# sxontheway/milliEye

Hardware: AMD Instinct MI355X
Metric: frames/sec YOLOv3-416+fusion @batch32, 1/2/4/8 MI355X; mAP@0.5 vs ref (higher is better)
Workload: dtype f32; 1 GPU; yolov3.cfg 416x416 fp32 inference, batch=32 per GPU, full milliEye: Darknet.forward -> NMS -> Network.forward mode 0 (R-CNN head + radar fusion, 2 radar boxes/frame) -> output rows, synthetic frames U[0,1), deterministic trained-like weights; stage=full, batch_per_gpu=32, global_batch=32, img_size=416, parallelism=frames sharded over 1 GPU(s), one process per GPU, no data-path collective, rccl_ranks=0, full=False, output_rows_last_step=6449, rois_last_step=6449

## Files before the change

### millieye_amd/csrc/common.h

```cpp
#pragma once
#include <hip/hip_runtime.h>
#include <stdint.h>
#include <stdio.h>
#include <stdlib.h>
#include "millieye_hip.h"

namespace me {

void set_error(const char* fmt, ...);

inline int check_launch(const char* what) {
  hipError_t e = hipGetLastError();
  if (e != hipSuccess) {
    set_error("%s: %s", what, hipGetErrorString(e));
    return (int)e;
  }
  return 0;
}

inline bool aligned16(const void* p) { return (reinterpret_cast<uintptr_t>(p) & 15u) == 0; }

inline int64_t ceil_div(int64_t a, int64_t b) { return (a + b - 1) / b; }

inline int store_mode() {
  static const int mode = [] {
    const char* e = getenv("MILLIEYE_STORE_MODE");
    return e ? atoi(e) : 0;
  }();
  return mode;
}

inline int epilogue16() {
  static const int on = [] {
    const char* e = getenv("MILLIEYE_EPILOGUE16");
    return e ? atoi(e) != 0 : 1;
  }();
  return on;
}

typedef unsigned st_u32x4 __attribute__((ext_vector_type(4)));
__device__ __forceinline__ void store16(void* ptr, uint4 v, int mode) {
  if (mode == 0) {
    *reinterpret_cast<uint4*>(ptr) = v;
  } else {
    st_u32x4 d = {v.x, v.y, v.z, v.w};
    if (mode == 1)
      asm volatile("global_store_dwordx4 %0, %1, off nt\n\ts_nop 1" ::"v"(ptr), "v"(d) : "memory");
    else
      asm volatile("global_store_dwordx4 %0, %1, off sc1\n\ts_nop 1" ::"v"(ptr), "v"(d) : "memory");
  }
}
__device__ __forceinline__ void store4(float* ptr, float v, int mode) {
  if (mode == 0)
    *ptr = v;
  else
    __builtin_nontemporal_store(v, ptr);
}

inline me_yolo_rect_desc yolo_rect_of(const me_yolo_desc& s) {
  me_yolo_rect_desc r;
  r.x = s.x;
  r.out = s.out;
  r.x_pitch = s.x_pitch;
  r.n = s.n;
  r.gh = r.gw = s.g;
  r.num_anchors = s.num_anchors;
  r.num_classes = s.num_classes;
  r.rows_total = s.rows_total;
  r.row_offset = s.row_offset;
  r.stride = s.stride;
  for (int i = 0; i < 16; ++i) r.anchors[i] = s.anchors[i];
  return r;
}

}

#define ME_REQUIRE(cond, code, ...)   \
  do {                                \
    if (!(cond)) {                    \
      me::set_error(__VA_ARGS__);     \
      return (code);                  \
    }                                 \
  } while (0)

#define ME_HIP(call)                                                 \
  do {                                                               \
    hipError_t e__ = (call);                                         \
// ... 6 lines not shown
```

### millieye_amd/csrc/conv.hip

```cpp
#include <stdlib.h>

#include "common.h"
#include "dma.h"

#include "conv32_common.h"

namespace me32 {
int launch_p8_tile(const ConvP& p, int tile, hipStream_t stream);
bool ws1x1_f32_eligible(const ConvP& p);
int launch_ws1x1_f32(const ConvP& p, hipStream_t stream);
bool ws3x3_f32_eligible(const ConvP& p);
int launch_ws3x3_f32(const ConvP& p, hipStream_t stream);
bool stem_mfma_eligible(const ConvP& p);
int launch_stem_mfma(const ConvP& p, hipStream_t stream);
}

namespace {

template <int BM, int BN, int BK, int WR, int WC, int ABL = 0, int PRIO = 0>
__global__ __launch_bounds__(256) void conv_igemm_f32(ConvP p) {
  static_assert(WR * WC == 4, "4 waves per workgroup");
  constexpr int TM = BM / WR, TN = BN / WC;
  constexpr int MT = TM / 32, NT = TN / 32;
  static_assert(MT >= 1 && NT >= 1, "wave tile must hold at least one 32x32 MFMA tile");
// ... 426 lines not shown
    for (int kx = 0; kx < 3; ++kx) {
      const int iy = oy * p.stride - p.pad + ky, ix = ox * p.stride - p.pad + kx;
      const bool ok = ((unsigned)iy < (unsigned)p.h) && ((unsigned)ix < (unsigned)p.w);
#pragma unroll
      for (int c = 0; c < 3; ++c) {
        float v = 0.f;
        if (ok)
          v = p.x_nchw ? p.x[(((long long)nimg * 3 + c) * p.h + iy) * p.w + ix]
                       : p.x[((long long)(nimg * p.h + iy) * p.w + ix) * p.x_pitch + c];
        xin[(ky * 3 + kx) * 3 + c] = v;
      }
    }
  const float* __restrict__ wg = p.wgt + (long long)co0 * K;
  float acc[CT];
#pragma unroll
  for (int j = 0; j < CT; ++j) {
    float a = 0.f;
#pragma unroll
    for (int k = 0; k < K; ++k) a = fmaf(xin[k], wg[j * K + k], a);
    acc[j] = apply_act(a * p.scale[co0 + j] + p.shift[co0 + j], p.act);
  }
  float* yrow = p.y + (long long)m * p.y_pitch + co0;
#pragma unroll
  for (int j = 0; j < CT; j += 4) *reinterpret_cast<float4*>(yrow + j) = make_float4(acc[j], acc[j + 1], acc[j + 2], acc[j + 3]);
}

using namespace me_dma;

__device__ __forceinline__ unsigned udiv_magic32(unsigned n, unsigned m, unsigned s) { return (__umulhi(n, m) + n) >> s; }

template <int N, class F, int I = 0>
__device__ __forceinline__ void static_for(F&& f) {
  if constexpr (I < N) {
    f(std::integral_constant<int, I>{});
    static_for<N, F, I + 1>(static_cast<F&&>(f));
  }
}

__device__ __forceinline__ void tile_coords(const ConvP& p, int t, int& tile_m, int& tile_n) {
  const int per_panel = p.tiles_m * p.gn;
  const int panel = t / per_panel;
  const int r = t - panel * per_panel;
  const int left = p.tiles_n - panel * p.gn;
  const int width = left < p.gn ? left : p.gn;
  tile_m = r / width;
  tile_n = panel * p.gn + (r - tile_m * width);
}

constexpr int buf_min_waves(int bm, int bn, int wr, int wc, int minw, bool hyb_or_masked) {
  const int per_wave = (bm / wr) * (bn / wc);
  return minw != 1 ? minw : per_wave == 1024 ? 6 : per_wave == 2048 && hyb_or_masked ? 4 : 1;
}

template <int BM, int BN, int WR, int WC, int MINW = 1, int BABL = 0, int HYB = 0, int KORD = 0, int DEEP = 0, int MASKED = 0>
__global__ __launch_bounds__(64 * WR * WC, buf_min_waves(BM, BN, WR, WC, MINW, HYB || MASKED)) void conv_igemm_buf_f32(ConvP p) {
  constexpr int NW = WR * WC;
  static_assert(NW == 4 || NW == 8, "4 or 8 waves per workgroup");
  constexpr int BK = 16, NST = DEEP ? (KORD ? 9 : 6) : 3;
  constexpr int DEPTH = NST - 1;
  constexpr int TM = BM / WR, TN = BN / WC;
  constexpr int MT = TM / 32, NT = TN / 32;
  constexpr int GA = BM / 16, G = (BM + BN) / 16;
  constexpr int LPW = (G + NW - 1) / NW;
  constexpr int LA = GA / NW;
  constexpr int STAGE_F = LPW * NW * 256;
  static_assert(GA % NW == 0, "A groups must split evenly over the waves");

  extern __shared__ __attribute__((aligned(16))) float smem[];
  const unsigned lds_base = (unsigned)(unsigned long long)(__attribute__((address_space(3))) float*)smem;

  const int tid = threadIdx.x;
  const int lane = tid & 63;
  const int wave = __builtin_amdgcn_readfirstlane(tid >> 6);
  const int wr = wave / WC, wc = wave % WC;
  const int r32 = lane & 31, hh = lane >> 5;

  int tile_m, tile_n;
  int sid = blockIdx.y;
  int piece = -1;
  {
    int nwg = p.tiles_m * p.tiles_n;
    int bid = blockIdx.x;
    int first = 0, per = 1;
    if constexpr (HYB) {
      if (bid < p.bulk) {
        nwg = p.bulk;
      } else {
        bid -= p.bulk;
        first = p.bulk;
        per = p.splitk;
        nwg = (nwg - p.bulk) * p.splitk;
      }
    }
    const int q = nwg >> 3, r = nwg & 7;
    const int xcd = bid & 7, idx = bid >> 3;
    int wg = (xcd < r ? xcd * (q + 1) : r * (q + 1) + (xcd - r) * q) + idx;
    if constexpr (HYB) {
      if (first || p.bulk == 0) {
        piece = wg;
        sid = wg % per;
        wg = first + wg / per;
      } else {
        sid = 0;
      }
    }
    tile_coords(p, wg, tile_m, tile_n);
    tile_m = __builtin_amdgcn_readfirstlane(tile_m);
    tile_n = __builtin_amdgcn_readfirstlane(tile_n);
  }
  const int m0 = tile_m * BM, n0 = tile_n * BN;
  const int hw = p.ho * p.wo;

  const int img0 = (int)udiv_magic32((unsigned)m0, p.hw_m, p.hw_s);
  const long long img_elems = (long long)p.h * p.w * p.x_pitch;
  const long long bias_elems = ((long long)p.pad * p.w + p.pad) * p.x_pitch;
  const u32x4 rsrc_a = make_rsrc(p.x + (long long)img0 * img_elems - bias_elems);
  const bool b_tiled = p.wgt_tiled != nullptr;
  const u32x4 rsrc_b = make_rsrc(b_tiled ? p.wgt_tiled + (long long)n0 * 16 : p.wgt + (long long)n0 * p.ktot);
  const unsigned b_row = b_tiled ? 64u : (unsigned)p.ktot * 4u;
  const unsigned b_step = b_tiled ? (unsigned)p.cout * 64u : BK * 4u;

  const int lrow = lane >> 2;
  unsigned v_base[LPW];
  constexpr bool KS3 = KORD == 1;
  unsigned v_pad[LA];
  unsigned v_cur[LPW];
#pragma unroll
  for (int j = 0; j < LPW; ++j) {
    const int g = wave + NW * j;
    const int row = g * 16 + lrow;
    const int q = (lane & 3) ^ ((row >> 2) & 3);
    v_base[j] = kOobOffset;
    if (j < LA) {
      unsigned padmask = 0xFFFFFFFFu;
      const int m = m0 + row;
      if (m < p.M) {
        const int nimg = (int)udiv_magic32((unsigned)m, p.hw_m, p.hw_s);
        const int rem = m - nimg * hw;
        const int oy = (int)udiv_magic32((unsigned)rem, p.wo_m, p.wo_s), ox = rem - oy * p.wo;
        const int iy0 = oy * p.stride - p.pad, ix0 = ox * p.stride - p.pad;
        unsigned ok = 0;
        auto in_w = [&](int kx) { return (unsigned)(ix0 + kx) < (unsigned)p.w ? 1u : 0u; };
        auto in_h = [&](int ky) { return (unsigned)(iy0 + ky) < (unsigned)p.h; };
        if (KS3 || p.ks == 3) {
          const unsigned cols = in_w(0) | in_w(1) << 1 | in_w(2) << 2;
          ok = (in_h(0) ? cols : 0u) | (in_h(1) ? cols << 3 : 0u) | (in_h(2) ? cols << 6 : 0u);
        } else if (p.ks == 1) {
          ok = in_h(0) ? in_w(0) : 0u;
        } else {
          unsigned cols = 0;
          for (int kx = 0; kx < p.ks; ++kx) cols |= in_w(kx) << kx;
          for (int ky = 0; ky < p.ks; ++ky) ok |= (in_h(ky) ? cols : 0u) << (ky * p.ks);
        }
        padmask = ~ok;
        const long long e = (long long)(nimg - img0) * img_elems + ((long long)iy0 * p.w + ix0) * p.x_pitch + bias_elems;
        v_base[j] = (unsigned)(e * 4) + 16u * q;
      }
      v_pad[j] = padmask;
    } else if (g < G) {
      const int co_local = row - BM;
      if (n0 + co_local < p.cout) v_base[j] = (unsigned)co_local * b_row + 16u * q;
    }
    v_cur[j] = BABL == 1 ? kOobOffset : v_base[j];
  }

  int s_begin = sid * p.sps;
  int s_end = (s_begin + p.sps < p.stages) ? s_begin + p.sps : p.stages;
  if constexpr (HYB) {
    if (piece < 0) {
      s_begin = 0;
      s_end = p.stages;
    }
  }
  f32x16 acc[MT][NT];
#pragma unroll
  for (int i = 0; i < MT; ++i)
#pragma unroll
    for (int j = 0; j < NT; ++j)
#pragma unroll
      for (int e = 0; e < 16; ++e) acc[i][j][e] = 0.f;

  constexpr unsigned STAGE_B = STAGE_F * 4u;
  const unsigned wave_lds = __builtin_amdgcn_readfirstlane(lds_base + (unsigned)wave * 1024u);
  const unsigned pitch4 = (unsigned)p.x_pitch * 4u;
  const int sw = (r32 >> 2) & 3;
  const int off0 = ((0 + hh) ^ sw) * 4, off1 = ((2 + hh) ^ sw) * 4;
  const float* a_frag = smem + (wr * TM + r32) * BK;
  const float* b_frag = smem + (BM + wc * TN + r32) * BK;

  auto compute_stage = [&](const float* Ab, const float* Bb) {
    if (MT * NT >= 4) __builtin_amdgcn_s_setprio(1);
    float4 af[2][MT], bf[2][NT];
#pragma unroll
    for (int half = 0; half < 2; ++half) {
      const int off = half ? off1 : off0;
#pragma unroll
      for (int i = 0; i < MT; ++i) af[half][i] = *reinterpret_cast<const float4*>(Ab + i * 32 * BK + off);
#pragma unroll
      for (int j = 0; j < NT; ++j) bf[half][j] = *reinterpret_cast<const float4*>(Bb + j * 32 * BK + off);
    }
    __builtin_amdgcn_sched_barrier(0);
#pragma unroll
    for (int half = 0; half < 2; ++half) {
#pragma unroll
      for (int kk = 0; kk < 4; ++kk)
#pragma unroll
        for (int i = 0; i < MT; ++i)
#pragma unroll
          for (int j = 0; j < NT; ++j) {
            const float4 av = af[half][i], bv = bf[half][j];
            const float a = kk == 0 ? av.x : kk == 1 ? av.y : kk == 2 ? av.z : av.w;
            const float b = kk == 0 ? bv.x : kk == 1 ? bv.y : kk == 2 ? bv.z : bv.w;
            acc[i][j] = __builtin_amdgcn_mfma_f32_32x32x2f32(a, b, acc[i][j], 0, 0, 0);
          }
    }
    if (MT * NT >= 4) __builtin_amdgcn_s_setprio(0);
  };

  if constexpr (KORD == 0) {
    int tap = 0, cc = 0, ky = 0, kx = 0;
    unsigned tmask = 0xFFFFFFFFu;
    if constexpr (MASKED) {
      tmask = p.tapmask[n0 / p.mask_cols] & ((1u << (p.ks * p.ks)) - 1u);
      tap = __builtin_ctz(tmask);
      ky = tap / p.ks;
      kx = tap - ky * p.ks;
      s_begin = 0;
      s_end = __builtin_popcount(tmask) * p.cs;
    } else if (s_begin != 0) {
      tap = s_begin / p.cs;
      cc = s_begin - tap * p.cs;
      ky = tap / p.ks;
      kx = tap - ky * p.ks;
    }
    unsigned a_off = 0, b_off = 0;
    auto enter_tap = [&]() {
#pragma unroll
      for (int j = 0; j < LA; ++j) v_cur[j] = (BABL == 1 || ((v_pad[j] >> (MASKED ? (tap & 31) : tap)) & 1u)) ? kOobOffset : v_base[j];
      a_off = (unsigned)(ky * p.w + kx) * pitch4;
      b_off = (unsigned)tap * (unsigned)p.cs * b_step;
    };
    enter_tap();
    a_off += (unsigned)cc * (BK * 4u);
    b_off += (unsigned)cc * b_step;
    auto issue_stage = [&](unsigned lds_dst) {
      dma_stage<LPW, LA, NW * 1024>(v_cur, rsrc_a, rsrc_b, __builtin_amdgcn_readfirstlane(a_off),
                                    __builtin_amdgcn_readfirstlane(b_off), lds_dst);
      a_off += BK * 4u;
      b_off += b_step;
      if (++cc == p.cs) {
        cc = 0;
        do {
          ++tap;
          if (++kx == p.ks) {
            kx = 0;
            ++ky;
          }
        } while (MASKED && tap < p.ks * p.ks && !((tmask >> tap) & 1u));
        enter_tap();
      }
    };
    const int nstages = s_end - s_begin;
    for (int i = 0; i < DEPTH && i < nstages; ++i) issue_stage(wave_lds + (unsigned)i * STAGE_B);
    auto wait_landed = [&](int younger) {
      bool done = false;
      static_for<DEPTH>([&](auto r_c) {
        constexpr int R = decltype(r_c)::value;
        if (!done && younger <= R) {
          asm volatile("s_waitcnt vmcnt(%0) lgkmcnt(0)" ::"n"(LPW * R) : "memory");
          done = true;
        }
      });
      if (!done) asm volatile("s_waitcnt vmcnt(%0) lgkmcnt(0)" ::"n"(LPW * (DEPTH - 1)) : "memory");
    };
    auto step = [&](auto slot_c) {
      constexpr int SLOT = decltype(slot_c)::value;
      asm volatile("s_waitcnt vmcnt(%0) lgkmcnt(0)" ::"n"(LPW * (DEPTH - 1)) : "memory");
      __builtin_amdgcn_s_barrier();
      asm volatile("" ::: "memory");
      issue_stage(wave_lds + ((SLOT + DEPTH) % NST) * STAGE_B);
      compute_stage(a_frag + SLOT * STAGE_F, b_frag + SLOT * STAGE_F);
    };
    int s = 0;
    for (; s + NST <= nstages - DEPTH; s += NST) static_for<NST>(step);
    int slot = 0;
    for (; s < nstages; ++s) {
      wait_landed(nstages - 1 - s);
      __builtin_amdgcn_s_barrier();
      asm volatile("" ::: "memory");
      if (s + DEPTH < nstages) issue_stage(wave_lds + (slot == 0 ? NST - 1 : slot - 1) * STAGE_B);
      compute_stage(a_frag + slot * STAGE_F, b_frag + slot * STAGE_F);
      slot = slot == NST - 1 ? 0 : slot + 1;
    }
  } else {
    unsigned v_tap[9][LPW];
    unsigned a_tap[9], b_tap[9];
#pragma unroll
    for (int t = 0; t < 9; ++t) {
#pragma unroll
      for (int j = 0; j < LPW; ++j)
        v_tap[t][j] = j < LA ? ((BABL == 1 || ((v_pad[j < LA ? j : 0] >> t) & 1u)) ? kOobOffset : v_base[j]) : v_cur[j];
      a_tap[t] = (unsigned)((t / 3) * p.w + (t % 3)) * pitch4;
      b_tap[t] = (unsigned)t * (unsigned)p.cs * b_step;
    }
    const int c_begin = s_begin / 9, c_end = s_end / 9;
    unsigned ca = (unsigned)c_begin * (BK * 4u), cb = (unsigned)c_begin * b_step;
    auto issue = [&](auto tap_c, unsigned ca_, unsigned cb_, unsigned lds_dst) {
      constexpr int T = decltype(tap_c)::value;
      dma_stage<LPW, LA, NW * 1024>(v_tap[T], rsrc_a, rsrc_b, __builtin_amdgcn_readfirstlane(a_tap[T] + ca_),
                                    __builtin_amdgcn_readfirstlane(b_tap[T] + cb_), lds_dst);
    };
    auto step = [&](auto tap_c, auto last_c) {
      constexpr int T = decltype(tap_c)::value;
      constexpr bool LAST = decltype(last_c)::value;
      constexpr int SLOT = T % NST;
      constexpr int YOUNGER = (LAST && 8 - T < DEPTH - 1) ? 8 - T : DEPTH - 1;
      asm volatile("s_waitcnt vmcnt(%0) lgkmcnt(0)" ::"n"(LPW * YOUNGER) : "memory");
      __builtin_amdgcn_s_barrier();
      asm volatile("" ::: "memory");
      constexpr unsigned DST = ((SLOT + DEPTH) % NST) * STAGE_B;
      if constexpr (T + DEPTH < 9)
        issue(std::integral_constant<int, (T + DEPTH) % 9>{}, ca, cb, wave_lds + DST);
      else if constexpr (!LAST)
        issue(std::integral_constant<int, (T + DEPTH) % 9>{}, ca + BK * 4u, cb + b_step, wave_lds + DST);
      compute_stage(a_frag + SLOT * STAGE_F, b_frag + SLOT * STAGE_F);
    };
    auto chunk = [&](auto last_c) { static_for<9>([&](auto tap_c) { step(tap_c, last_c); }); };
    static_for<DEPTH>([&](auto tap_c) { issue(tap_c, ca, cb, wave_lds + decltype(tap_c)::value * STAGE_B); });
    for (int c = c_begin; c + 1 < c_end; ++c) {
      chunk(std::false_type{});
      ca += BK * 4u;
      cb += b_step;
    }
    chunk(std::true_type{});
  }

  const bool split = HYB ? piece >= 0 : p.splitk > 1;
  if (split) {
    const long long slab_stride = HYB ? (long long)(BM * BN) : (long long)p.M * p.cout;
    float* slab0 = HYB ? p.partial + (long long)(piece - sid) * (BM * BN) : p.partial;
    auto slab_index = [&](int i, int j, int e, long long& idx) {
      const int lm = wr * TM + i * 32 + (e & 3) + 8 * (e >> 2) + 4 * hh, lc = wc * TN + j * 32 + r32;
      if (HYB) {
        idx = (long long)lm * BN + lc;
        return true;
      }
      idx = (long long)(m0 + lm) * p.cout + (n0 + lc);
      return m0 + lm < p.M && n0 + lc < p.cout;
    };
    float* mine = slab0 + (long long)sid * slab_stride;
#pragma unroll
    for (int j = 0; j < NT; ++j)
#pragma unroll
      for (int i = 0; i < MT; ++i)
#pragma unroll
        for (int e = 0; e < 16; ++e) {
          long long idx;
          if (!slab_index(i, j, e, idx)) continue;
          if (p.counters)
            __hip_atomic_store(mine + idx, acc[i][j][e], __ATOMIC_RELAXED, __HIP_MEMORY_SCOPE_AGENT);
          else
            mine[idx] = acc[i][j][e];
        }
    if (p.counters == nullptr) return;
    asm volatile("s_waitcnt vmcnt(0)" ::: "memory");
    __syncthreads();
    int* last_flag = reinterpret_cast<int*>(smem);
    if (tid == 0) {
      int* cnt = p.counters + (HYB ? piece / p.splitk : tile_m * p.tiles_n + tile_n);
      const int ticket = __hip_atomic_fetch_add(cnt, 1, __ATOMIC_RELAXED, __HIP_MEMORY_SCOPE_AGENT);
      const int last = ticket == p.splitk - 1;
      if (last) __hip_atomic_store(cnt, 0, __ATOMIC_RELAXED, __HIP_MEMORY_SCOPE_AGENT);
      *last_flag = last;
    }
    __syncthreads();
    if (*last_flag == 0) return;
#pragma unroll
    for (int j = 0; j < NT; ++j)
#pragma unroll
      for (int i = 0; i < MT; ++i)
#pragma unroll
        for (int e = 0; e < 16; ++e) {
          long long idx;
          if (!slab_index(i, j, e, idx)) continue;
          float a = __hip_atomic_load(slab0 + idx, __ATOMIC_RELAXED, __HIP_MEMORY_SCOPE_AGENT);
// ... 385 lines not shown
      attr_set = true;
    }
  }
  const long long blocks = (long long)p.tiles_m * p.tiles_n;
  ME_REQUIRE(blocks < (1ll << 31), ME_E_TOOBIG, "me_conv2d_f32: grid too large");
  hipLaunchKernelGGL(kern, dim3((unsigned)blocks, (unsigned)p.splitk), dim3(256), lds, stream, p);
  int rc = me::check_launch("conv_igemm_f32");
  if (rc || p.splitk == 1) return rc;
  long long rb = ((long long)p.M * p.cout + 255) / 256;
  if (rb > 256 * 16) rb = 256 * 16;
  hipLaunchKernelGGL(conv_splitk_reduce_f32, dim3((unsigned)rb), dim3(256), 0, stream, p);
  return me::check_launch("conv_splitk_reduce_f32");
}

template <int BM, int BN, int WR, int WC, int DPRIO = 0, int MINW = 1, int DABL = 0>
int launch_dma(ConvP& p, hipStream_t stream) {
  ME_REQUIRE(p.ks * p.ks <= 32, ME_E_BADARG, "conv_igemm_dma_f32: filters larger than 5x5 need the register-staged tiles (51-55)");
  constexpr int BK = 16;
  p.cs = (p.cin + BK - 1) / BK;
  p.stages = p.ks * p.ks * p.cs;
  p.tiles_m = (p.M + BM - 1) / BM;
  p.tiles_n = (p.cout + BN - 1) / BN;
  plan_split(p);
  constexpr int NW = WR * WC;
  constexpr int LPW = ((BM + BN) / 16 + NW - 1) / NW;
  const size_t lds = (size_t)3 * LPW * NW * 256 * sizeof(float);
  auto kern = conv_igemm_dma_f32<BM, BN, WR, WC, DPRIO, MINW, DABL>;
  if (lds > 64 * 1024) {
    static bool attr_set = false;
    if (!attr_set) {
      ME_HIP(hipFuncSetAttribute(reinterpret_cast<const void*>(kern), hipFuncAttributeMaxDynamicSharedMemorySize,
                                 (int)lds));
      attr_set = true;
    }
  }
  const long long blocks = (long long)p.tiles_m * p.tiles_n;
  ME_REQUIRE(blocks < (1ll << 31), ME_E_TOOBIG, "me_conv2d_f32: grid too large");
  hipLaunchKernelGGL(kern, dim3((unsigned)blocks, (unsigned)p.splitk), dim3(64 * NW), lds, stream, p);
  int rc = me::check_launch("conv_igemm_dma_f32");
  if (rc || p.splitk == 1) return rc;
  long long rb = ((long long)p.M * p.cout + 255) / 256;
  if (rb > 256 * 16) rb = 256 * 16;
  hipLaunchKernelGGL(conv_splitk_reduce_f32, dim3((unsigned)rb), dim3(256), 0, stream, p);
  return me::check_launch("conv_splitk_reduce_f32");
}

template <int BM>
bool buf_addressable(const ConvP& p) {
  if (p.cin % 16 != 0 || p.x_nchw) return false;
  const long long hw = (long long)p.ho * p.wo;
  const long long span_imgs = (BM - 1) / hw + 2;
  const long long img_bytes = (long long)p.h * p.w * p.x_pitch * 4;
  const long long tap_bytes = ((long long)p.ks * p.w + p.ks) * p.x_pitch * 4 + (long long)p.cin * 4;
  const long long a_max = span_imgs * img_bytes + 2 * tap_bytes;
  const long long b_max = 256ll * p.ktot * 4 + (long long)p.ktot * 4;
  const long long b_tiled_max = p.wgt_tiled ? (long long)p.ktot * p.cout * 4 + 256ll * 64 : 0;
  return a_max < (1ll << 31) && b_max < (1ll << 31) && b_tiled_max < (1ll << 31) && (long long)p.x_pitch * 4 < (1ll << 31);
}

void magic_u32(unsigned d, unsigned* m, unsigned* s) {
  unsigned sh = 0;
  while ((1ull << sh) < d) ++sh;
  *s = sh;
  *m = (unsigned)(((1ull << 32) * ((1ull << sh) - d)) / d + 1);
}

template <int BN>
void choose_order(ConvP& p) {
  static const long long kPanelBytes = [] {
    const char* e = getenv("MILLIEYE_PANEL_KB");
    return (e && atoi(e) > 0 ? (long long)atoi(e) : 1300ll) * 1024;
  }();
  static const int kChunkMajor = [] {
    const char* e = getenv("MILLIEYE_KORD");
    return e ? atoi(e) : 2;
  }();
  const long long col_bytes = (long long)BN * p.ktot * 4;
  p.gn = p.tiles_n;
  p.kord = (p.ks == 3 && p.cs >= 4 && kChunkMajor == 2) ? 1 : 0;
  if (col_bytes * p.tiles_n > kPanelBytes) {
    const long long fit = kPanelBytes / col_bytes;
    p.gn = fit < 1 ? 1 : fit > p.tiles_n ? p.tiles_n : (int)fit;
    if (p.ks == 3 && kChunkMajor >= 1) p.kord = 1;
  }
}

template <int BM, int BN, int WR, int WC, int MINW, int BABL, int HYB, int KORD, int DEEP = 0, int MASKED = 0>
int launch_buf_kernel(const ConvP& p, dim3 grid, hipStream_t stream) {
  constexpr int NW = WR * WC;
  constexpr int LPW = ((BM + BN) / 16 + NW - 1) / NW;
  constexpr int NST = DEEP ? (KORD ? 9 : 6) : 3;
  const size_t lds = (size_t)NST * LPW * NW * 256 * sizeof(float);
  auto kern = conv_igemm_buf_f32<BM, BN, WR, WC, MINW, BABL, HYB, KORD, DEEP, MASKED>;
  if (lds > 64 * 1024) {
    static bool attr_set = false;
    if (!attr_set) {
      ME_HIP(hipFuncSetAttribute(reinterpret_cast<const void*>(kern), hipFuncAttributeMaxDynamicSharedMemorySize,
                                 (int)lds));
      attr_set = true;
    }
  }
  hipLaunchKernelGGL(kern, grid, dim3(64 * NW), lds, stream, p);
  return me::check_launch(HYB ? "conv_igemm_buf_f32<tail split>" : "conv_igemm_buf_f32");
}

template <int BM, int BN, int WR, int WC, int MINW = 1, int BABL = 0, int DEEP = 0>
int launch_buf(ConvP& p, hipStream_t stream) {
  if (p.ks * p.ks > 32) {
    if constexpr (WR * WC == 4)
      return launch_igemm<BM, BN, 16, WR, WC>(p, stream);
    else
      return launch_igemm<128, 128, 16, 2, 2>(p, stream);
  }
  if (p.mask_cols)
    ME_REQUIRE(buf_addressable<BM>(p) && p.mask_cols % BN == 0 && BABL == 0 && DEEP == 0, ME_E_BADARG,
               "me_conv2d_f32: tap masks need cin %% 16 == 0, offsets below 2^31 and a tile width (%d) that divides tap_mask_cols", BN);
  if (!buf_addressable<BM>(p)) return launch_dma<BM, BN, WR, WC, 1, MINW>(p, stream);
  constexpr int BK = 16;
  p.cs = (p.cin + BK - 1) / BK;
  p.stages = p.ks * p.ks * p.cs;
  p.tiles_m = (p.M + BM - 1) / BM;
  p.tiles_n = (p.cout + BN - 1) / BN;
  choose_order<BN>(p);
  if (BABL || p.mask_cols) p.kord = 0;
  plan_split(p);
  const long long blocks = (long long)p.tiles_m * p.tiles_n;
  ME_REQUIRE(blocks < (1ll << 31), ME_E_TOOBIG, "me_conv2d_f32: grid too large");
  const dim3 grid((unsigned)blocks, (unsigned)p.splitk);
  if (blocks > p.counters_len || p.splitk == 1) p.counters = nullptr;
  int rc;
  if constexpr (BABL == 0) {
    if (p.mask_cols) {
      if constexpr (DEEP == 0) rc = launch_buf_kernel<BM, BN, WR, WC, MINW, 0, 0, 0, 0, 1>(p, grid, stream);
      else rc = ME_E_BADARG;
    } else
      rc = p.kord ? launch_buf_kernel<BM, BN, WR, WC, MINW, 0, 0, 1, DEEP>(p, grid, stream)
                  : launch_buf_kernel<BM, BN, WR, WC, MINW, 0, 0, 0, DEEP>(p, grid, stream);
  } else {
    rc = launch_buf_kernel<BM, BN, WR, WC, MINW, BABL, 0, 0>(p, grid, stream);
  }
  if (rc || p.splitk == 1 || p.counters) return rc;
  long long rb = ((long long)p.M * p.cout + 255) / 256;
  if (rb > 256 * 16) rb = 256 * 16;
  hipLaunchKernelGGL(conv_splitk_reduce_f32, dim3((unsigned)rb), dim3(256), 0, stream, p);
  return me::check_launch("conv_splitk_reduce_f32");
}

template <int BM, int BN, int WR, int WC, int MINW = 1, int DEEP = 0>
int launch_buf_tail(ConvP& p, hipStream_t stream, long long ws_bytes) {
  ME_REQUIRE(p.ks * p.ks <= 32 && buf_addressable<BM>(p), ME_E_BADARG,
             "me_conv2d_f32: the tail-split tiles need cin %% 16 == 0 and offsets below 2^31");
  constexpr int BK = 16;
  p.cs = (p.cin + BK - 1) / BK;
  p.stages = p.ks * p.ks * p.cs;
  p.tiles_m = (p.M + BM - 1) / BM;
  p.tiles_n = (p.cout + BN - 1) / BN;
  choose_order<BN>(p);
  const long long tiles = (long long)p.tiles_m * p.tiles_n;
  ME_REQUIRE(tiles < (1ll << 24), ME_E_TOOBIG, "me_conv2d_f32: grid too large");
  plan_split(p);
  p.bulk = (int)(tiles / 256 * 256);
  const long long tail = tiles - p.bulk;
  if (tail == 0 || p.splitk <= 1) {
    p.splitk = 1;
    p.bulk = 0;
    return launch_buf<BM, BN, WR, WC, MINW, 0, DEEP>(p, stream);
  }
  const long long need = tail * p.splitk * BM * BN * (long long)sizeof(float);
  ME_REQUIRE(p.partial && ws_bytes >= need, ME_E_BADARG, "me_conv2d_f32: tail split %d needs a workspace of %lld bytes",
             p.splitk, need);
  const dim3 grid((unsigned)(p.bulk + tail * p.splitk));
  if (tail > p.counters_len) p.counters = nullptr;
  int rc = p.kord ? launch_buf_kernel<BM, BN, WR, WC, MINW, 0, 1, 1, DEEP>(p, grid, stream)
                  : launch_buf_kernel<BM, BN, WR, WC, MINW, 0, 1, 0, DEEP>(p, grid, stream);
  if (rc || p.counters) return rc;
  long long rb = (tail * BM * BN + 255) / 256;
  if (rb > 256 * 16) rb = 256 * 16;
  hipLaunchKernelGGL(conv_tail_reduce_f32, dim3((unsigned)rb), dim3(256), 0, stream, p, BM, BN);
  return me::check_launch("conv_tail_reduce_f32");
}

int fill_params(const me_conv_desc* d, ConvP& p) {
  p.store_mode = me::store_mode();
  ME_REQUIRE(d != nullptr, ME_E_NULLPTR, "me_conv2d_f32: null descriptor");
  ME_REQUIRE(d->n > 0 && d->h > 0 && d->w > 0 && d->cin > 0 && d->cout > 0, ME_E_BADARG,
             "me_conv2d_f32: non-positive dimension");
  ME_REQUIRE(d->ksize >= 1 && d->stride >= 1 && d->pad >= 0, ME_E_BADARG, "me_conv2d_f32: bad ksize/stride/pad");
  const int ho = (d->h + 2 * d->pad - d->ksize) / d->stride + 1;
  const int wo = (d->w + 2 * d->pad - d->ksize) / d->stride + 1;
  ME_REQUIRE(ho == d->ho && wo == d->wo, ME_E_BADARG, "me_conv2d_f32: ho/wo (%d,%d) != derived (%d,%d)", d->ho,
             d->wo, ho, wo);
  ME_REQUIRE((long long)d->n * d->ho * d->wo < (1ll << 31), ME_E_TOOBIG, "me_conv2d_f32: too many output pixels");
  p.x = d->x; p.wgt = d->wgt; p.wgt_tiled = d->wgt_tiled; p.scale = d->scale; p.shift = d->shift; p.res = d->res; p.y = d->y;
  p.x_pitch = d->x_pitch; p.res_pitch = d->res_pitch; p.y_pitch = d->y_pitch;
  p.n = d->n; p.h = d->h; p.w = d->w; p.cin = d->cin; p.cout = d->cout; p.ks = d->ksize;
  p.stride = d->stride; p.pad = d->pad; p.ho = d->ho; p.wo = d->wo; p.act = d->act; p.ups = d->upsample;
  p.x_nchw = d->x_nchw;
  p.M = d->n * d->ho * d->wo;
  p.ktot = d->ksize * d->ksize * d->cin;
  magic_u32((unsigned)(d->ho * d->wo), &p.hw_m, &p.hw_s);
  magic_u32((unsigned)d->wo, &p.wo_m, &p.wo_s);
  p.cs = p.stages = p.tiles_m = p.tiles_n = p.bulk = p.gn = p.kord = 0;
  p.partial = nullptr;
  p.splitk = 1;
  p.sps = 0;
  p.counters = d->tile_counters_len > 0 ? d->tile_counters : nullptr;
  p.counters_len = p.counters ? d->tile_counters_len : 0;
  p.mask_cols = d->tap_mask_cols > 0 ? d->tap_mask_cols : 0;
  for (int i = 0; i < 4; ++i) p.tapmask[i] = d->tap_mask[i];
  auto rows16 = [](const float* ptr, long long pitch) { return me::aligned16(ptr) && pitch % 4 == 0 && pitch < (1ll << 22); };
  p.ep16 = me::epilogue16() && d->upsample == 1 && d->act != ME_ACT_SIGMOID && rows16(d->y, d->y_pitch) &&
           (!d->res || rows16(d->res, d->res_pitch)) && me::aligned16(d->scale) && me::aligned16(d->shift);
  return 0;
}

}

extern "C" {

int64_t me_conv2d_flops(const me_conv_desc* d) {
  if (!d) return 0;
  return 2ll * d->n * d->ho * d->wo * (int64_t)d->cout * d->ksize * d->ksize * d->cin;
}

int64_t me_conv2d_workspace_bytes(const me_conv_desc* d) {
  ConvP p;
  if (!d || fill_params(d, p) != 0 || d->cin <= 4) return 0;
// ... 145 lines not shown
```

### millieye_amd/csrc/dma.h

```cpp
#pragma once
#include <hip/hip_runtime.h>

namespace me_dma {

typedef unsigned u32x4 __attribute__((ext_vector_type(4)));
constexpr unsigned kOobOffset = 0x80000000u;

__device__ __forceinline__ u32x4 make_rsrc(const void* base) {
  const unsigned long long b = (unsigned long long)base;
  u32x4 r;
  r.x = __builtin_amdgcn_readfirstlane((unsigned)b);
  r.y = __builtin_amdgcn_readfirstlane((unsigned)(b >> 32) & 0xffffu);
  r.z = kOobOffset;
  r.w = 0x00020000u;
  return r;
}

template <int LPW, int LA, int STEP>
__device__ __forceinline__ void dma_stage(const unsigned (&v)[LPW], u32x4 ra, u32x4 rb, unsigned sa, unsigned sb,
                                          unsigned dst) {
  static_assert(LPW >= 2 && LPW <= 4 && LA >= 1 && LA <= 2, "unsupported DMA shape");
#define ME_DMA_HEAD "s_mov_b32 m0, %[d]\n\ts_nop 0\n\t"
#define ME_DMA_NEXT "s_add_u32 m0, m0, %[st]\n\ts_nop 0\n\t"
#define ME_DMA_A(i) "buffer_load_dwordx4 %[v" #i "], %[ra], %[sa] offen lds\n\t"
#define ME_DMA_B(i) "buffer_load_dwordx4 %[v" #i "], %[rb], %[sb] offen lds\n\t"
#define ME_DMA_TAIL ""
  if constexpr (LPW == 4 && LA == 2) {
    asm volatile(ME_DMA_HEAD ME_DMA_A(0) ME_DMA_NEXT ME_DMA_A(1) ME_DMA_NEXT ME_DMA_B(2) ME_DMA_NEXT ME_DMA_B(3) ME_DMA_TAIL
                 :
                 : [d] "s"(dst), [st] "n"(STEP), [ra] "s"(ra), [rb] "s"(rb), [sa] "s"(sa), [sb] "s"(sb), [v0] "v"(v[0]),
                   [v1] "v"(v[1]), [v2] "v"(v[2]), [v3] "v"(v[3])
                 : "memory", "scc");
  } else if constexpr (LPW == 3 && LA == 2) {
    asm volatile(ME_DMA_HEAD ME_DMA_A(0) ME_DMA_NEXT ME_DMA_A(1) ME_DMA_NEXT ME_DMA_B(2) ME_DMA_TAIL
                 :
                 : [d] "s"(dst), [st] "n"(STEP), [ra] "s"(ra), [rb] "s"(rb), [sa] "s"(sa), [sb] "s"(sb), [v0] "v"(v[0]),
                   [v1] "v"(v[1]), [v2] "v"(v[2])
                 : "memory", "scc");
  } else if constexpr (LPW == 2 && LA == 1) {
    asm volatile(ME_DMA_HEAD ME_DMA_A(0) ME_DMA_NEXT ME_DMA_B(1) ME_DMA_TAIL
                 :
                 : [d] "s"(dst), [st] "n"(STEP), [ra] "s"(ra), [rb] "s"(rb), [sa] "s"(sa), [sb] "s"(sb), [v0] "v"(v[0]),
                   [v1] "v"(v[1])
                 : "memory", "scc");
  } else {
    static_assert(LPW == 0, "add the (LPW, LA) combination");
  }
#undef ME_DMA_HEAD
#undef ME_DMA_NEXT
#undef ME_DMA_A
#undef ME_DMA_B
#undef ME_DMA_TAIL
}


template <int N, int STEP, int OFF, int LEN>
__device__ __forceinline__ void dma_same(const unsigned (&va)[LEN], u32x4 r, unsigned s, unsigned dst) {
  unsigned keep;
  static_assert(N >= 1 && N <= 4 && OFF + N <= LEN, "1..4 loads per block, inside the array");
  unsigned v[4];
#pragma unroll
  for (int i = 0; i < 4; ++i) v[i] = va[OFF + (i < N ? i : 0)];
#define ME_DMA_HEAD "s_mov_b32 %[k], m0\n\ts_mov_b32 m0, %[d]\n\ts_nop 0\n\t"
#define ME_DMA_NEXT "s_add_u32 m0, m0, %[st]\n\ts_nop 0\n\t"
#define ME_DMA_L(i) "buffer_load_dwordx4 %[v" #i "], %[r], %[s] offen lds\n\t"
#define ME_DMA_TAIL "s_mov_b32 m0, %[k]"
  if constexpr (N == 1) {
    asm volatile(ME_DMA_HEAD ME_DMA_L(0) ME_DMA_TAIL
                 : [k] "=&s"(keep)
                 : [d] "s"(dst), [st] "n"(STEP), [r] "s"(r), [s] "s"(s), [v0] "v"(v[0])
                 : "memory", "scc");
  } else if constexpr (N == 2) {
    asm volatile(ME_DMA_HEAD ME_DMA_L(0) ME_DMA_NEXT ME_DMA_L(1) ME_DMA_TAIL
                 : [k] "=&s"(keep)
// ... 22 lines not shown
```

Before: 1943 frames/s.

## Lean DMA loop: adjacent LDS slots with immediate offsets and rsrc-walking addressing

Reorganizes each wave's LDS slots so its load groups are contiguous, letting the buffer_load-to-LDS sequence use immediate offsets instead of m0 increments with s_nop. A new KORD=2 path for 1x1 stride-1 convs skips per-row padding math and walks the buffer resource base forward, using a fully unrolled ring schedule. The 3x3 chunk-major path also advances the resource descriptor instead of adding SGPR offsets. It adds template variants and an env switch (on by default), and widens the offset-range guard to reserve room for the immediates.

```diff
diff --git a/millieye_amd/csrc/common.h b/millieye_amd/csrc/common.h
--- a/millieye_amd/csrc/common.h
+++ b/millieye_amd/csrc/common.h
@@ -33,6 +33,14 @@
 inline int epilogue16() {
   static const int on = [] {
     const char* e = getenv("MILLIEYE_EPILOGUE16");
+    return e ? atoi(e) != 0 : 1;
+  }();
+  return on;
+}
+
+inline int lean_loop() {
+  static const int on = [] {
+    const char* e = getenv("MILLIEYE_LEAN_LOOP");
     return e ? atoi(e) != 0 : 1;
   }();
   return on;
diff --git a/millieye_amd/csrc/conv.hip b/millieye_amd/csrc/conv.hip
--- a/millieye_amd/csrc/conv.hip
+++ b/millieye_amd/csrc/conv.hip
@@ -502,11 +502,21 @@
   return minw != 1 ? minw : per_wave == 1024 ? 6 : per_wave == 2048 && hyb_or_masked ? 4 : 1;
 }
 
+constexpr bool buf_chunk_major(int kord) { return kord == 1 || kord == 3; }
+constexpr bool buf_adjacent(int kord) { return kord <= 2; }
+constexpr int buf_ring(int kord, int deep) { return deep ? (buf_chunk_major(kord) ? 9 : 6) : 3; }
+
+__device__ __forceinline__ void rsrc_advance(u32x4& r, unsigned bytes) {
+  const unsigned long long b = (((unsigned long long)r.y << 32) | r.x) + bytes;
+  r.x = __builtin_amdgcn_readfirstlane((unsigned)b);
+  r.y = __builtin_amdgcn_readfirstlane((unsigned)(b >> 32));
+}
+
 template <int BM, int BN, int WR, int WC, int MINW = 1, int BABL = 0, int HYB = 0, int KORD = 0, int DEEP = 0, int MASKED = 0>
 __global__ __launch_bounds__(64 * WR * WC, buf_min_waves(BM, BN, WR, WC, MINW, HYB || MASKED)) void conv_igemm_buf_f32(ConvP p) {
   constexpr int NW = WR * WC;
   static_assert(NW == 4 || NW == 8, "4 or 8 waves per workgroup");
-  constexpr int BK = 16, NST = DEEP ? (KORD ? 9 : 6) : 3;
+  constexpr int BK = 16, NST = buf_ring(KORD, DEEP);
   constexpr int DEPTH = NST - 1;
   constexpr int TM = BM / WR, TN = BN / WC;
   constexpr int MT = TM / 32, NT = TN / 32;
@@ -515,6 +525,9 @@
   constexpr int LA = GA / NW;
   constexpr int STAGE_F = LPW * NW * 256;
   static_assert(GA % NW == 0, "A groups must split evenly over the waves");
+  constexpr bool ADJ = buf_adjacent(KORD);
+  static_assert(!ADJ || (NW % (2 * MT) == 0 && NW % (2 * NT) == 0), "a wave's fragment groups must not wrap round the waves");
+  constexpr int GSTR = ADJ ? LPW : 1;
 
   extern __shared__ __attribute__((aligned(16))) float smem[];
   const unsigned lds_base = (unsigned)(unsigned long long)(__attribute__((address_space(3))) float*)smem;
@@ -564,15 +577,17 @@
   const int img0 = (int)udiv_magic32((unsigned)m0, p.hw_m, p.hw_s);
   const long long img_elems = (long long)p.h * p.w * p.x_pitch;
   const long long bias_elems = ((long long)p.pad * p.w + p.pad) * p.x_pitch;
-  const u32x4 rsrc_a = make_rsrc(p.x + (long long)img0 * img_elems - bias_elems);
+  constexpr int A_IMM = ADJ ? 1024 * (LA - 1) : 0, B_IMM = ADJ ? 1024 * (LPW - 1) : 0;
+  u32x4 rsrc_a = make_rsrc(reinterpret_cast<const char*>(p.x + (long long)img0 * img_elems - bias_elems) - A_IMM);
   const bool b_tiled = p.wgt_tiled != nullptr;
-  const u32x4 rsrc_b = make_rsrc(b_tiled ? p.wgt_tiled + (long long)n0 * 16 : p.wgt + (long long)n0 * p.ktot);
+  u32x4 rsrc_b = make_rsrc(reinterpret_cast<const char*>(b_tiled ? p.wgt_tiled + (long long)n0 * 16 : p.wgt + (long long)n0 * p.ktot) - B_IMM);
   const unsigned b_row = b_tiled ? 64u : (unsigned)p.ktot * 4u;
   const unsigned b_step = b_tiled ? (unsigned)p.cout * 64u : BK * 4u;
 
   const int lrow = lane >> 2;
   unsigned v_base[LPW];
-  constexpr bool KS3 = KORD == 1;
+  constexpr bool KS3 = buf_chunk_major(KORD);
+  constexpr bool KS1 = KORD == 2;
   unsigned v_pad[LA];
   unsigned v_cur[LPW];
 #pragma unroll
@@ -584,7 +599,12 @@
     if (j < LA) {
       unsigned padmask = 0xFFFFFFFFu;
       const int m = m0 + row;
-      if (m < p.M) {
+      if (KS1 && p.stride == 1) {
+        if (m < p.M) {
+          padmask = 0;
+          v_base[j] = (unsigned)(m - img0 * hw) * ((unsigned)p.x_pitch * 4u) + 16u * q + (unsigned)(A_IMM - (ADJ ? 1024 * j : 0));
+        }
+      } else if (m < p.M) {
         const int nimg = (int)udiv_magic32((unsigned)m, p.hw_m, p.hw_s);
         const int rem = m - nimg * hw;
         const int oy = (int)udiv_magic32((unsigned)rem, p.wo_m, p.wo_s), ox = rem - oy * p.wo;
@@ -604,12 +624,12 @@
         }
         padmask = ~ok;
         const long long e = (long long)(nimg - img0) * img_elems + ((long long)iy0 * p.w + ix0) * p.x_pitch + bias_elems;
-        v_base[j] = (unsigned)(e * 4) + 16u * q;
+        v_base[j] = (unsigned)(e * 4) + 16u * q + (unsigned)(A_IMM - (ADJ ? 1024 * j : 0));
       }
       v_pad[j] = padmask;
     } else if (g < G) {
       const int co_local = row - BM;
-      if (n0 + co_local < p.cout) v_base[j] = (unsigned)co_local * b_row + 16u * q;
+      if (n0 + co_local < p.cout) v_base[j] = (unsigned)co_local * b_row + 16u * q + (unsigned)(B_IMM - (ADJ ? 1024 * j : 0));
     }
     v_cur[j] = BABL == 1 ? kOobOffset : v_base[j];
   }
@@ -631,12 +651,17 @@
       for (int e = 0; e < 16; ++e) acc[i][j][e] = 0.f;
 
   constexpr unsigned STAGE_B = STAGE_F * 4u;
-  const unsigned wave_lds = __builtin_amdgcn_readfirstlane(lds_base + (unsigned)wave * 1024u);
+  const unsigned wave_lds = __builtin_amdgcn_readfirstlane(lds_base + (unsigned)wave * (ADJ ? LPW * 1024u : 1024u));
   const unsigned pitch4 = (unsigned)p.x_pitch * 4u;
   const int sw = (r32 >> 2) & 3;
   const int off0 = ((0 + hh) ^ sw) * 4, off1 = ((2 + hh) ^ sw) * 4;
-  const float* a_frag = smem + (wr * TM + r32) * BK;
-  const float* b_frag = smem + (BM + wc * TN + r32) * BK;
+  auto frag = [&](int row0) {
+    const int g0 = row0 >> 4;
+    const int slot = ADJ ? (g0 % NW) * LPW + g0 / NW : g0;
+    return smem + ((slot + (r32 >> 4) * GSTR) * 16 + (r32 & 15)) * BK;
+  };
+  const float* a_frag = frag(wr * TM);
+  const float* b_frag = frag(BM + wc * TN);
 
   auto compute_stage = [&](const float* Ab, const float* Bb) {
     if (MT * NT >= 4) __builtin_amdgcn_s_setprio(1);
@@ -645,9 +670,9 @@
     for (int half = 0; half < 2; ++half) {
       const int off = half ? off1 : off0;
 #pragma unroll
-      for (int i = 0; i < MT; ++i) af[half][i] = *reinterpret_cast<const float4*>(Ab + i * 32 * BK + off);
-#pragma unroll
-      for (int j = 0; j < NT; ++j) bf[half][j] = *reinterpret_cast<const float4*>(Bb + j * 32 * BK + off);
+      for (int i = 0; i < MT; ++i) af[half][i] = *reinterpret_cast<const float4*>(Ab + i * GSTR * 32 * BK + off);
+#pragma unroll
+      for (int j = 0; j < NT; ++j) bf[half][j] = *reinterpret_cast<const float4*>(Bb + j * GSTR * 32 * BK + off);
     }
     __builtin_amdgcn_sched_barrier(0);
 #pragma unroll
@@ -667,7 +692,7 @@
     if (MT * NT >= 4) __builtin_amdgcn_s_setprio(0);
   };
 
-  if constexpr (KORD == 0) {
+  if constexpr (KORD == 0 || KORD == 4) {
     int tap = 0, cc = 0, ky = 0, kx = 0;
     unsigned tmask = 0xFFFFFFFFu;
     if constexpr (MASKED) {
@@ -694,7 +719,7 @@
     a_off += (unsigned)cc * (BK * 4u);
     b_off += (unsigned)cc * b_step;
     auto issue_stage = [&](unsigned lds_dst) {
-      dma_stage<LPW, LA, NW * 1024>(v_cur, rsrc_a, rsrc_b, __builtin_amdgcn_readfirstlane(a_off),
+      dma_stage<LPW, LA, NW * 1024, ADJ>(v_cur, rsrc_a, rsrc_b, __builtin_amdgcn_readfirstlane(a_off),
                                     __builtin_amdgcn_readfirstlane(b_off), lds_dst);
       a_off += BK * 4u;
       b_off += b_step;
@@ -742,6 +767,46 @@
       compute_stage(a_frag + slot * STAGE_F, b_frag + slot * STAGE_F);
       slot = slot == NST - 1 ? 0 : slot + 1;
     }
+  } else if constexpr (KS1) {
+    const int nstages = s_end - s_begin;
+    rsrc_advance(rsrc_a, (unsigned)s_begin * (BK * 4u));
+    rsrc_advance(rsrc_b, (unsigned)s_begin * b_step);
+    unsigned kb[NST];
+#pragma unroll
+    for (int k = 0; k < NST; ++k) kb[k] = (unsigned)k * b_step;
+    const unsigned trip_b = (unsigned)NST * b_step;
+    auto issue = [&](auto k_c) {
+      constexpr int K = decltype(k_c)::value;
+      if constexpr (K == 0) {
+        rsrc_advance(rsrc_a, NST * BK * 4u);
+        rsrc_advance(rsrc_b, trip_b);
+      }
+      dma_stage<LPW, LA, NW * 1024, ADJ>(v_cur, rsrc_a, rsrc_b, __builtin_amdgcn_readfirstlane((unsigned)K * (BK * 4u)),
+                                    __builtin_amdgcn_readfirstlane(kb[K]), wave_lds + K * STAGE_B);
+    };
+    auto last_step = [&](auto i_c, auto r_c) {
+      constexpr int I = decltype(i_c)::value, R = decltype(r_c)::value;
+      constexpr int SLOT = I % NST;
+      constexpr int YOUNGER = R - 1 - I < DEPTH - 1 ? R - 1 - I : DEPTH - 1;
+      asm volatile("s_waitcnt vmcnt(%0) lgkmcnt(0)" ::"n"(LPW * YOUNGER) : "memory");
+      __builtin_amdgcn_s_barrier();
+      asm volatile("" ::: "memory");
+      if constexpr (I + DEPTH < R) issue(std::integral_constant<int, (I + DEPTH) % NST>{});
+      compute_stage(a_frag + SLOT * STAGE_F, b_frag + SLOT * STAGE_F);
+    };
+    auto step = [&](auto slot_c) { last_step(slot_c, std::integral_constant<int, NST + DEPTH>{}); };
+#pragma unroll
+    for (int i = 0; i < DEPTH; ++i)
+      if (i < nstages)
+        dma_stage<LPW, LA, NW * 1024, ADJ>(v_cur, rsrc_a, rsrc_b, __builtin_amdgcn_readfirstlane((unsigned)i * (BK * 4u)),
+                                      __builtin_amdgcn_readfirstlane(kb[i]), wave_lds + (unsigned)i * STAGE_B);
+    int s = 0;
+    for (; s + NST <= nstages - DEPTH; s += NST) static_for<NST>(step);
+    const int left = nstages - s;
+    static_for<NST + DEPTH - 1>([&](auto r_c) {
+      constexpr int R = decltype(r_c)::value + 1;
+      if (left == R) static_for<R>([&](auto i_c) { last_step(i_c, std::integral_constant<int, R>{}); });
+    });
   } else {
     unsigned v_tap[9][LPW];
     unsigned a_tap[9], b_tap[9];
@@ -754,11 +819,21 @@
       b_tap[t] = (unsigned)t * (unsigned)p.cs * b_step;
     }
     const int c_begin = s_begin / 9, c_end = s_end / 9;
+    constexpr bool LEAN = KORD == 1;
     unsigned ca = (unsigned)c_begin * (BK * 4u), cb = (unsigned)c_begin * b_step;
+    if constexpr (LEAN) {
+      rsrc_advance(rsrc_a, ca);
+      rsrc_advance(rsrc_b, cb);
+      ca = cb = 0;
+    }
     auto issue = [&](auto tap_c, unsigned ca_, unsigned cb_, unsigned lds_dst) {
       constexpr int T = decltype(tap_c)::value;
-      dma_stage<LPW, LA, NW * 1024>(v_tap[T], rsrc_a, rsrc_b, __builtin_amdgcn_readfirstlane(a_tap[T] + ca_),
-                                    __builtin_amdgcn_readfirstlane(b_tap[T] + cb_), lds_dst);
+      if constexpr (LEAN)
+        dma_stage<LPW, LA, NW * 1024, ADJ>(v_tap[T], rsrc_a, rsrc_b, __builtin_amdgcn_readfirstlane(a_tap[T]),
+                                      __builtin_amdgcn_readfirstlane(b_tap[T]), lds_dst);
+      else
+        dma_stage<LPW, LA, NW * 1024, ADJ>(v_tap[T], rsrc_a, rsrc_b, __builtin_amdgcn_readfirstlane(a_tap[T] + ca_),
+                                      __builtin_amdgcn_readfirstlane(b_tap[T] + cb_), lds_dst);
     };
     auto step = [&](auto tap_c, auto last_c) {
       constexpr int T = decltype(tap_c)::value;
@@ -769,6 +844,10 @@
       __builtin_amdgcn_s_barrier();
       asm volatile("" ::: "memory");
       constexpr unsigned DST = ((SLOT + DEPTH) % NST) * STAGE_B;
+      if constexpr (LEAN && !LAST && T + DEPTH == 9) {
+        rsrc_advance(rsrc_a, BK * 4u);
+        rsrc_advance(rsrc_b, b_step);
+      }
       if constexpr (T + DEPTH < 9)
         issue(std::integral_constant<int, (T + DEPTH) % 9>{}, ca, cb, wave_lds + DST);
       else if constexpr (!LAST)
@@ -779,8 +858,10 @@
     static_for<DEPTH>([&](auto tap_c) { issue(tap_c, ca, cb, wave_lds + decltype(tap_c)::value * STAGE_B); });
     for (int c = c_begin; c + 1 < c_end; ++c) {
       chunk(std::false_type{});
-      ca += BK * 4u;
-      cb += b_step;
+      if constexpr (!LEAN) {
+        ca += BK * 4u;
+        cb += b_step;
+      }
     }
     chunk(std::true_type{});
   }
@@ -1272,9 +1353,10 @@
   const long long span_imgs = (BM - 1) / hw + 2;
   const long long img_bytes = (long long)p.h * p.w * p.x_pitch * 4;
   const long long tap_bytes = ((long long)p.ks * p.w + p.ks) * p.x_pitch * 4 + (long long)p.cin * 4;
-  const long long a_max = span_imgs * img_bytes + 2 * tap_bytes;
-  const long long b_max = 256ll * p.ktot * 4 + (long long)p.ktot * 4;
-  const long long b_tiled_max = p.wgt_tiled ? (long long)p.ktot * p.cout * 4 + 256ll * 64 : 0;
+  const long long kImmRoom = 4096;
+  const long long a_max = span_imgs * img_bytes + 2 * tap_bytes + kImmRoom;
+  const long long b_max = 256ll * p.ktot * 4 + (long long)p.ktot * 4 + kImmRoom;
+  const long long b_tiled_max = p.wgt_tiled ? (long long)p.ktot * p.cout * 4 + 256ll * 64 + kImmRoom : 0;
   return a_max < (1ll << 31) && b_max < (1ll << 31) && b_tiled_max < (1ll << 31) && (long long)p.x_pitch * 4 < (1ll << 31);
 }
 
@@ -1309,7 +1391,7 @@
 int launch_buf_kernel(const ConvP& p, dim3 grid, hipStream_t stream) {
   constexpr int NW = WR * WC;
   constexpr int LPW = ((BM + BN) / 16 + NW - 1) / NW;
-  constexpr int NST = DEEP ? (KORD ? 9 : 6) : 3;
+  constexpr int NST = buf_ring(KORD, DEEP);
   const size_t lds = (size_t)NST * LPW * NW * 256 * sizeof(float);
   auto kern = conv_igemm_buf_f32<BM, BN, WR, WC, MINW, BABL, HYB, KORD, DEEP, MASKED>;
   if (lds > 64 * 1024) {
@@ -1322,6 +1404,18 @@
   }
   hipLaunchKernelGGL(kern, grid, dim3(64 * NW), lds, stream, p);
   return me::check_launch(HYB ? "conv_igemm_buf_f32<tail split>" : "conv_igemm_buf_f32");
+}
+
+template <int BM, int BN, int WR, int WC, int MINW, int HYB, int DEEP>
+int launch_buf_kernel_walk(const ConvP& p, dim3 grid, hipStream_t stream) {
+  const bool lean = me::lean_loop() != 0;
+  if (p.kord)
+    return lean ? launch_buf_kernel<BM, BN, WR, WC, MINW, 0, HYB, 1, DEEP>(p, grid, stream)
+                : launch_buf_kernel<BM, BN, WR, WC, MINW, 0, HYB, 3, DEEP>(p, grid, stream);
+  if constexpr ((BM / WR) * (BN / WC) == 1024)
+    if (lean && p.ks == 1 && p.pad == 0) return launch_buf_kernel<BM, BN, WR, WC, MINW, 0, HYB, 2, DEEP>(p, grid, stream);
+  return lean ? launch_buf_kernel<BM, BN, WR, WC, MINW, 0, HYB, 0, DEEP>(p, grid, stream)
+              : launch_buf_kernel<BM, BN, WR, WC, MINW, 0, HYB, 4, DEEP>(p, grid, stream);
 }
 
 template <int BM, int BN, int WR, int WC, int MINW = 1, int BABL = 0, int DEEP = 0>
@@ -1351,11 +1445,12 @@
   int rc;
   if constexpr (BABL == 0) {
     if (p.mask_cols) {
-      if constexpr (DEEP == 0) rc = launch_buf_kernel<BM, BN, WR, WC, MINW, 0, 0, 0, 0, 1>(p, grid, stream);
+      if constexpr (DEEP == 0)
+        rc = me::lean_loop() ? launch_buf_kernel<BM, BN, WR, WC, MINW, 0, 0, 0, 0, 1>(p, grid, stream)
+                             : launch_buf_kernel<BM, BN, WR, WC, MINW, 0, 0, 4, 0, 1>(p, grid, stream);
       else rc = ME_E_BADARG;
     } else
-      rc = p.kord ? launch_buf_kernel<BM, BN, WR, WC, MINW, 0, 0, 1, DEEP>(p, grid, stream)
-                  : launch_buf_kernel<BM, BN, WR, WC, MINW, 0, 0, 0, DEEP>(p, grid, stream);
+      rc = launch_buf_kernel_walk<BM, BN, WR, WC, MINW, 0, DEEP>(p, grid, stream);
   } else {
     rc = launch_buf_kernel<BM, BN, WR, WC, MINW, BABL, 0, 0>(p, grid, stream);
   }
@@ -1391,8 +1486,7 @@
              p.splitk, need);
   const dim3 grid((unsigned)(p.bulk + tail * p.splitk));
   if (tail > p.counters_len) p.counters = nullptr;
-  int rc = p.kord ? launch_buf_kernel<BM, BN, WR, WC, MINW, 0, 1, 1, DEEP>(p, grid, stream)
-                  : launch_buf_kernel<BM, BN, WR, WC, MINW, 0, 1, 0, DEEP>(p, grid, stream);
+  int rc = launch_buf_kernel_walk<BM, BN, WR, WC, MINW, 1, DEEP>(p, grid, stream);
   if (rc || p.counters) return rc;
   long long rb = (tail * BM * BN + 255) / 256;
   if (rb > 256 * 16) rb = 256 * 16;
diff --git a/millieye_amd/csrc/dma.h b/millieye_amd/csrc/dma.h
--- a/millieye_amd/csrc/dma.h
+++ b/millieye_amd/csrc/dma.h
@@ -16,10 +16,39 @@
   return r;
 }
 
-template <int LPW, int LA, int STEP>
+template <int LPW, int LA, int STEP, bool ADJ = false>
 __device__ __forceinline__ void dma_stage(const unsigned (&v)[LPW], u32x4 ra, u32x4 rb, unsigned sa, unsigned sb,
                                           unsigned dst) {
   static_assert(LPW >= 2 && LPW <= 4 && LA >= 1 && LA <= 2, "unsupported DMA shape");
+  if constexpr (ADJ) {
+#define ME_DMA_HEAD "s_mov_b32 m0, %[d]\n\ts_nop 0\n\t"
+#define ME_DMA_A(i, imm) "buffer_load_dwordx4 %[v" #i "], %[ra], %[sa] offen" imm " lds\n\t"
+#define ME_DMA_B(i, imm) "buffer_load_dwordx4 %[v" #i "], %[rb], %[sb] offen" imm " lds\n\t"
+    if constexpr (LPW == 4 && LA == 2) {
+      asm volatile(ME_DMA_HEAD ME_DMA_A(0, "") ME_DMA_A(1, " offset:1024") ME_DMA_B(2, " offset:2048") ME_DMA_B(3, " offset:3072")
+                   :
+                   : [d] "s"(dst), [ra] "s"(ra), [rb] "s"(rb), [sa] "s"(sa), [sb] "s"(sb), [v0] "v"(v[0]), [v1] "v"(v[1]),
+                     [v2] "v"(v[2]), [v3] "v"(v[3])
+                   : "memory");
+    } else if constexpr (LPW == 3 && LA == 2) {
+      asm volatile(ME_DMA_HEAD ME_DMA_A(0, "") ME_DMA_A(1, " offset:1024") ME_DMA_B(2, " offset:2048")
+                   :
+                   : [d] "s"(dst), [ra] "s"(ra), [rb] "s"(rb), [sa] "s"(sa), [sb] "s"(sb), [v0] "v"(v[0]), [v1] "v"(v[1]),
+                     [v2] "v"(v[2])
+                   : "memory");
+    } else if constexpr (LPW == 2 && LA == 1) {
+      asm volatile(ME_DMA_HEAD ME_DMA_A(0, "") ME_DMA_B(1, " offset:1024")
+                   :
+                   : [d] "s"(dst), [ra] "s"(ra), [rb] "s"(rb), [sa] "s"(sa), [sb] "s"(sb), [v0] "v"(v[0]), [v1] "v"(v[1])
+                   : "memory");
+    } else {
+      static_assert(LPW == 0, "add the (LPW, LA) combination");
+    }
+#undef ME_DMA_HEAD
+#undef ME_DMA_A
+#undef ME_DMA_B
+    return;
+  }
 #define ME_DMA_HEAD "s_mov_b32 m0, %[d]\n\ts_nop 0\n\t"
 #define ME_DMA_NEXT "s_add_u32 m0, m0, %[st]\n\ts_nop 0\n\t"
 #define ME_DMA_A(i) "buffer_load_dwordx4 %[v" #i "], %[ra], %[sa] offen lds\n\t"
```

New measurement: 1952 frames/s, median of 6. About the same (+0.4%).
